# locuoco/coulomb_oscillators

Hardware: AMD Instinct MI355X
Metric: particle-steps/sec (+ Gpair-interactions/sec), N=1048576 FMM-3D kd-tree p=6, 1 GPU(s) (higher is better)
Workload: dtype f32; 1 GPU; FMM-3D kd-tree p=6, N=1048576 per GPU (one system of 1048576), leapfrog, Gaussian ball, tree rebuilt every 1 step(s); n_per_gpu=1048576, order=6, parallelism=single GPU, L=15, p2p_pairs=3193446, m2l_pairs=800719, build_mode=0, warm_builds=283, warm_misses=12, near_field=one-directional

## Files before the change

### coulomb_oscillators_amd/csrc/k_fmm_kd.hip

```cpp
#include "nbco_internal.hpp"
#include "k_p2p.hpp"
#include "kd_common.hpp"
#include <rocprim/rocprim.hpp>
#include <chrono>
#include <functional>
#include <cmath>
#include <algorithm>
#include <vector>

namespace {

using kdc::wave_scan_add;
using kdc::wave_min_u32;

constexpr int sym_off(int n) { return n * (n + 1) * (n + 2) / 6; }
constexpr int tl_off(int n) { return n * n; }

struct TreeView
{
	float *center, *lbound, *rbound;
	float4 *csz;
	float *mpole, *local;
	int *mult, *index, *splitdim;
	int L, ntot;
// ... 137 lines not shown
		hipLaunchKernelGGL(list_segsort_kernel<false>, dim3((ntargets + kBlock / 64 - 1) / (kBlock / 64)), dim3(kBlock), 0, st, (const int *)start,
		                   ntargets, keys_tmp, keys_out, shift, (const int *)nullptr, (const int *)nullptr, (int2 *)nullptr, MutualLists{}, 0);
	NBCO_HIP(hipGetLastError());
	return NBCO_OK;
}

static int kd_carve(nbco_ctx *c, DevBuf &buf, KdTreeDev &k, int ntot, int offM, int offL)
{
	const size_t rb = c->o.far_fp64 ? 8 : 4;
	k.real_bytes = (int)rb;
	size_t bytes = (size_t)ntot * (3 * 3 * sizeof(float) + sizeof(float4) + (size_t)(offM + offL) * rb + 3 * sizeof(int)) + 256 + 64;
	NBCO_TRY(c->reserve(buf, bytes));
	char *q = (char *)buf.ptr;
	k.csz = (float4 *)q; q += sizeof(float4) * (size_t)ntot;
	k.center = (float *)q; q += 12 * (size_t)ntot;
	k.lbound = (float *)q; q += 12 * (size_t)ntot;
	k.rbound = (float *)q; q += 12 * (size_t)ntot;
	q = (char *)(((uintptr_t)q + 15) & ~(uintptr_t)15);
	k.mpole = (float *)q; q += rb * (size_t)ntot * offM;
	q = (char *)(((uintptr_t)q + 15) & ~(uintptr_t)15);
	k.local = (float *)q; q += rb * (size_t)ntot * offL;
	q = (char *)(((uintptr_t)q + 15) & ~(uintptr_t)15);
	k.mult = (int *)q; q += 4 * (size_t)ntot;
	k.index = (int *)q; q += 4 * (size_t)ntot;
	k.splitdim = (int *)q;
	return NBCO_OK;
}

static int kd_build_top(nbco_ctx *c, const TreeView &tv, float4 *&pos, float4 *&pos_alt, int *&unsort, int *&unsort_alt, long long n, int l0,
                        bool use_select, bool select_ready = false, bool warm = false)
{
	hipStream_t st = c->stream;
	if (use_select && l0 > 0 && !select_ready) NBCO_TRY(kd_select_begin(c, l0));
	for (int l = 0; l < l0; ++l)
	{
		if (use_select)
			NBCO_TRY(kd_select_level(c, l, n, pos, unsort, pos_alt, unsort_alt, tv.lbound, tv.rbound, tv.splitdim, tv.index,
			                         c->counters.as<int>() + 110, warm));
		else
		{
			if (l > 0) hipLaunchKernelGGL(kd_box_kernel, dim3(grid1d(kd_cnt(l))), dim3(kBlock), 0, st, tv, pos, n, l);
			hipLaunchKernelGGL(kd_keys_kernel, dim3(grid1d(n)), dim3(kBlock), 0, st, pos, tv.splitdim + kd_beg(l), n, l,
			                   c->keys.as<uint64_t>(), c->idx.as<uint32_t>());
			NBCO_TRY(sort_pairs_u64(c, c->keys.as<uint64_t>(), c->keys_alt.as<uint64_t>(), c->idx.as<uint32_t>(), c->idx_alt.as<uint32_t>(), n, 32 + l));
			hipLaunchKernelGGL(kd_permute_kernel, dim3(grid1d(n)), dim3(kBlock), 0, st, pos, unsort, c->idx_alt.as<uint32_t>(), pos_alt, unsort_alt, n);
		}
		std::swap(pos, pos_alt);
		std::swap(unsort, unsort_alt);
	}
	if (l0 > 0 && !use_select) hipLaunchKernelGGL(kd_box_kernel, dim3(grid1d(kd_cnt(l0))), dim3(kBlock), 0, st, tv, pos, n, l0);
	NBCO_HIP(hipGetLastError());
	return NBCO_OK;
}

static int kd_reserve_particles(nbco_ctx *c, long long n)
{
	NBCO_TRY(c->reserve(c->pos4, sizeof(float4) * (size_t)n));
	NBCO_TRY(c->reserve(c->pos4_alt, sizeof(float4) * (size_t)n));
	NBCO_TRY(c->reserve(c->unsort, sizeof(int) * (size_t)n));
	NBCO_TRY(c->reserve(c->unsort_alt, sizeof(int) * (size_t)n));
	NBCO_TRY(c->reserve(c->keys, sizeof(uint64_t) * (size_t)n));
	NBCO_TRY(c->reserve(c->keys_alt, sizeof(uint64_t) * (size_t)n));
	NBCO_TRY(c->reserve(c->idx, sizeof(uint32_t) * (size_t)n));
	NBCO_TRY(c->reserve(c->idx_alt, sizeof(uint32_t) * (size_t)n));
	NBCO_TRY(c->reserve(c->counters, sizeof(int) * 128));
	return NBCO_OK;
}

static int kd_build_upward(nbco_ctx *c, const float *p, long long n, int L, const float *root6, bool &rebuild, int stage = 0)
// ... 526 lines not shown
```

### coulomb_oscillators_amd/csrc/k_kdselect.hip

```cpp
#include "nbco_internal.hpp"
#include "kd_common.hpp"

namespace {

using namespace kdc;

constexpr int kBlockBig = 1024, kBlockSmall = 256;
constexpr int kBins = 2048;
constexpr int kTieCap = 64;
constexpr int kTieWords = 8;

struct SelNode
{
	uint32_t prefix[2], r[2];
	uint32_t done_part;
	uint32_t cntL, cntR, tiecnt;
	uint32_t minR;
	uint32_t below;
};

struct SelPivot { uint32_t prefix, r, neq, need; };

__device__ inline uint32_t ld_agent_u32(const uint32_t *p) { return __hip_atomic_load(p, __ATOMIC_RELAXED, __HIP_MEMORY_SCOPE_AGENT); }

template <int BLOCK>
__device__ inline void descend(const uint32_t *__restrict__ h, int bits, SelPivot &pv, uint32_t *sh )
{
	constexpr int R = BLOCK / 64;
	constexpr int PER = kBins / BLOCK;
	uint32_t v[PER], s = 0;
#pragma unroll
	for (int q = 0; q < PER; ++q) { v[q] = ld_agent_u32(&h[threadIdx.x * PER + q]); s += v[q]; }
	const int lane = threadIdx.x & 63, w = threadIdx.x >> 6;
	uint32_t incl = s;
	for (int o = 1; o < 64; o <<= 1) { uint32_t y = __shfl_up(incl, o); if (lane >= o) incl += y; }
	__syncthreads();
	if (lane == 63) sh[w] = incl;
	__syncthreads();
	uint32_t base = 0;
	for (int q = 0; q < w; ++q) base += sh[q];
	uint32_t cum = base + incl - s;
#pragma unroll
	for (int q = 0; q < PER; ++q)
	{
		if (pv.r >= cum && pv.r < cum + v[q]) { sh[R] = threadIdx.x * PER + q; sh[R + 1] = cum; sh[R + 2] = v[q]; }
		cum += v[q];
	}
	__syncthreads();
	pv.prefix = (pv.prefix << bits) | sh[R];
	pv.r -= sh[R + 1];
	pv.neq = sh[R + 2];
// ... 559 lines not shown
				uint32_t *rec = tielist + ((size_t)(j0 + jj) * kTieCap + t) * kTieWords;
				const int a2 = anc23[jj][0], a3 = anc23[jj][1];
				const uint32_t w[7] = {ordered_bits(axis_of(p[e], sd[jj])), a2 >= 0 ? ordered_bits(axis_of(p[e], a2)) : 0u,
				                       a3 >= 0 ? ordered_bits(axis_of(p[e], a3)) : 0u, (uint32_t)org[e],
				                       __float_as_uint(p[e].x), __float_as_uint(p[e].y), __float_as_uint(p[e].z)};
#pragma unroll
				for (int q = 0; q < 7; ++q) __hip_atomic_store(&rec[q], w[q], __ATOMIC_RELAXED, __HIP_MEMORY_SCOPE_AGENT);
			}
		}
		if (cat[e] < 0) continue;
		const int q = cat[e];
		const long long dst = (q == 0 ? first[0] : (q == 1 ? first[1] : (q == 2 ? first[2] : first[3])))
		                      + (long long)((pw[e * W + wv] >> (16 * q)) & 0xFFFF) + lp[e];
		pos_out[dst] = p[e];
		unsort_out[dst] = org[e];
	}
	__shared__ uint32_t fin[2];
	PART_MARK(6);
	asm volatile("s_waitcnt vmcnt(0)" ::: "memory");
	__syncthreads();
	PART_MARK(7);
	if (threadIdx.x < 2) fin[threadIdx.x] = (j0 + threadIdx.x <= j1) ? atomicAdd(&nodes[j0 + threadIdx.x].done_part, 1u) : 0xFFFFFFFFu;
	__syncthreads();
	PART_MARK(8);
	if (threadIdx.x < 64)
		for (int jj = 0; jj < 2; ++jj)
			if (j0 + jj <= j1 && fin[jj] == chunks_of_node<CHUNK>(n, j0 + jj, m) - 1)
				ties_and_boxes(pos_out, unsort_out, lbound, rbound, splitdim, index, nodes, tielist, flag, n, l, (int)(j0 + jj),
				               (int)threadIdx.x, pvs[jj], meta[jj]);
	PART_MARK(9);
}


}

int kd_select_begin(nbco_ctx *c, int l0, bool zero, long long *words_a, long long *words_b)
{
	const size_t nodes = ((size_t)1 << l0) - 1;
	NBCO_TRY(c->reserve(c->sel_hist, sizeof(uint32_t) * 3 * nodes * kBins));
	NBCO_TRY(c->reserve(c->sel_nodes, sizeof(SelNode) * nodes));
	NBCO_TRY(c->reserve(c->sel_ties, sizeof(uint32_t) * nodes * kTieCap * kTieWords));
	if (words_a) *words_a = (long long)(3 * nodes * kBins);
	if (words_b) *words_b = (long long)(sizeof(SelNode) / sizeof(uint32_t) * nodes);
	if (zero)
	{
		NBCO_HIP(hipMemsetAsync(c->sel_hist.ptr, 0, sizeof(uint32_t) * 3 * nodes * kBins, c->stream));
		NBCO_HIP(hipMemsetAsync(c->sel_nodes.ptr, 0, sizeof(SelNode) * nodes, c->stream));
	}
	return NBCO_OK;
}

template <int BLOCK, int NP>
static void select_level_launch(nbco_ctx *c, int l, long long n, const float4 *pos_in, const int *unsort_in, float4 *pos_out, int *unsort_out,
                                float *lbound, float *rbound, int *splitdim, int *index, int *flag, int warm_drop)
{
	const int m = 1 << l;
	SelNode *nodes = c->sel_nodes.as<SelNode>() + (m - 1);
	uint32_t *hist = c->sel_hist.as<uint32_t>() + (size_t)3 * (m - 1) * kBins;
	uint32_t *ties = c->sel_ties.as<uint32_t>() + (size_t)(m - 1) * kTieCap * kTieWords;
	const int *sd_l = splitdim + (m - 1);
	hipStream_t st = c->stream;
	constexpr int CHUNK = 8 * BLOCK;
	const int gchunks = (int)((n + CHUNK - 1) / CHUNK);
	if (NP == 2 && warm_drop > 0)
	{
		constexpr int EPT = BLOCK == kBlockBig ? 4 : 8;
		const int wchunks = (int)((n + EPT * BLOCK - 1) / (EPT * BLOCK));
		hipLaunchKernelGGL((sel_hist_warm_kernel<BLOCK, EPT>), dim3(wchunks), dim3(BLOCK), 0, st, pos_in, sd_l, hist, nodes, (const float *)lbound, (const float *)rbound,
		                   n, l, warm_drop);
		hipLaunchKernelGGL((sel_partition_kernel<BLOCK, 2, true, EPT>), dim3(wchunks), dim3(BLOCK), 0, st, pos_in, unsort_in, pos_out, unsort_out, sd_l, nodes, ties, n, l,
		                   lbound, rbound, splitdim, index, flag, (const uint32_t *)hist, warm_drop, c->top_sd, c->top_root1);
		return;
	}
	hipLaunchKernelGGL((sel_hist_kernel<0, BLOCK, NP == 2>), dim3(gchunks), dim3(BLOCK), 0, st, pos_in, sd_l, hist, nodes, (const float *)lbound, (const float *)rbound, n, l);
	hipLaunchKernelGGL((sel_hist_kernel<1, BLOCK, NP == 2>), dim3(gchunks), dim3(BLOCK), 0, st, pos_in, sd_l, hist, nodes, (const float *)lbound, (const float *)rbound, n, l);
	if (NP >= 3)
		hipLaunchKernelGGL((sel_hist_kernel<2, BLOCK, false>), dim3(gchunks), dim3(BLOCK), 0, st, pos_in, sd_l, hist, nodes, (const float *)lbound, (const float *)rbound, n, l);
	hipLaunchKernelGGL((sel_partition_kernel<BLOCK, NP>), dim3(gchunks), dim3(BLOCK), 0, st, pos_in, unsort_in, pos_out, unsort_out, sd_l, nodes, ties, n, l,
	                   lbound, rbound, splitdim, index, flag, (const uint32_t *)hist, 10, c->top_sd, c->top_root1);
}

int kd_select_level(nbco_ctx *c, int l, long long n, const float4 *pos_in, const int *unsort_in, float4 *pos_out, int *unsort_out,
                    float *lbound, float *rbound, int *splitdim, int *index, int *flag, bool warm)
{
	const long long node = n >> l;
	const int np = (c->sel_three_pass || node > (1LL << 22)) ? 3 : 2;
	const bool big = node >= 8 * kBlockBig;
	int warm_drop = 0;
	if (warm && np == 2)
	{
		int lg = 0;
		while ((1LL << lg) < node) ++lg;
		warm_drop = 32 - std::max(12, std::min(22, std::max(16, lg + 6)) - 2 * c->sel_warm_coarsen);
	}
#define NBCO_SEL_ARGS c, l, n, pos_in, unsort_in, pos_out, unsort_out, lbound, rbound, splitdim, index, flag, warm_drop
	if (big)
	{
		if (np == 2) select_level_launch<kBlockBig, 2>(NBCO_SEL_ARGS);
		else select_level_launch<kBlockBig, 3>(NBCO_SEL_ARGS);
	}
	else
	{
		if (np == 2) select_level_launch<kBlockSmall, 2>(NBCO_SEL_ARGS);
		else select_level_launch<kBlockSmall, 3>(NBCO_SEL_ARGS);
	}
#undef NBCO_SEL_ARGS
	NBCO_HIP(hipGetLastError());
	return NBCO_OK;
}
```

### coulomb_oscillators_amd/csrc/nbco_api.hip

```cpp
#include "nbco_internal.hpp"
#include <chrono>
#include <cstdio>
#include <cmath>
#include <new>
#include <random>

int nbco_ctx::reserve(DevBuf &b, size_t bytes)
{
	nbco_ctx *c = this;
	if (bytes <= b.bytes) return NBCO_OK;
	if (b.ptr)
	{
		NBCO_HIP(hipStreamSynchronize(stream));
		NBCO_HIP(hipFree(b.ptr));
		b.ptr = nullptr;
		b.bytes = 0;
	}
	size_t want = bytes + bytes / 8 + 256;
	NBCO_HIP(hipMalloc(&b.ptr, want));
	b.bytes = want;
	if (poison) NBCO_HIP(hipMemsetAsync(b.ptr, 0x7f, want, stream));
	return NBCO_OK;
}

// ... 111 lines not shown
	o->list_grow = 1;
	o->far_fp64 = 0;
	o->p2p_mutual = 0;
	o->track_order = 0;
	o->stream = nullptr;
	return NBCO_OK;
}

int nbco_create(nbco_ctx **out, const nbco_opts *o)
{
	if (!out) return NBCO_ERR_ARG;
	*out = nullptr;
	nbco_ctx *c = new (std::nothrow) nbco_ctx();
	if (!c) return NBCO_ERR_HIP;
	nbco_opts def;
	nbco_opts_default(&def);
	c->o = o ? *o : def;
	int rc = check_opts(c, &c->o);
	if (rc != NBCO_OK) { delete c; return rc; }
	int ndev = 0;
	hipError_t e = hipGetDeviceCount(&ndev);
	if (e != hipSuccess || ndev <= 0)
	{
		fprintf(stderr, "nbco_create: no usable HIP device (%s)\n", e != hipSuccess ? hipGetErrorString(e) : "device count is 0");
		delete c;
		return NBCO_ERR_HIP;
	}
	if (hipGetDevice(&c->device) != hipSuccess) { delete c; return NBCO_ERR_HIP; }
	hipDeviceProp_t prop;
	if (hipGetDeviceProperties(&prop, c->device) == hipSuccess) c->num_cu = prop.multiProcessorCount;
	c->stream = (hipStream_t)c->o.stream;
	c->poison = getenv("NBCO_POISON") && atoi(getenv("NBCO_POISON")) != 0;
	if (getenv("NBCO_SEL_WARM")) c->sel_warm_enabled = atoi(getenv("NBCO_SEL_WARM")) != 0;
	if (hipMalloc(&c->small.ptr, 4096) != hipSuccess) { delete c; return NBCO_ERR_HIP; }
	c->small.bytes = 4096;
	*out = c;
	return NBCO_OK;
}

int nbco_destroy(nbco_ctx *c)
{
	if (c && getenv("NBCO_HOST_TIMING") && c->host_calls)
		fprintf(stderr, "[nbco] nbco_integrate: %lld calls, %.1f us host time per call, of which %.1f us waiting for the traversal flags\n", c->host_calls,
		        1e6 * c->host_call_s / c->host_calls, 1e6 * c->host_wait_s / c->host_calls);
	if (!c) return NBCO_OK;
	hipStreamSynchronize(c->stream);
	DevBuf *bufs[] = {&c->pos4, &c->pos4_alt, &c->part, &c->small, &c->tmp3, &c->keys, &c->keys_alt, &c->idx, &c->idx_alt,
	                  &c->unsort, &c->unsort_alt, &c->sort_tmp, &c->treebuf, &c->frontier_a, &c->frontier_b, &c->p2p_list,
	                  &c->m2l_list, &c->counters, &c->p2p_keys, &c->p2p_keys_alt, &c->m2l_keys, &c->m2l_keys_alt,
	                  &c->p2p_start, &c->m2l_start, &c->p2p_chunk_off, &c->p2p_chunks, &c->sel_hist, &c->sel_nodes, &c->sel_ties, &c->list_cnt,
	                  &c->dist_top, &c->dist_tree, &c->oct_tree, &c->oct_groups, &c->scan_tmp_aux, &c->p2p_desc, &c->trav_ctr, &c->prep_state, &c->p2p_sec, &c->p2p_react, &c->order, &c->order_alt,
	                  &c->let_sel, &c->let_have, &c->dist_pos, &c->tmp3b, &c->dpart_buf};
	if (c->aux && !c->aux_is_main) { hipStreamSynchronize(c->aux); hipStreamDestroy(c->aux); }
	if (c->ev_fork) hipEventDestroy(c->ev_fork);
	if (c->ev_join) hipEventDestroy(c->ev_join);
	if (c->ev_flags) hipEventDestroy(c->ev_flags);
	if (c->h_flags) hipHostFree(c->h_flags);
	for (DevBuf *b : bufs)
		if (b->ptr) hipFree(b->ptr);
	for (auto &t : c->timers)
		for (auto &ev : t.pending) { hipEventDestroy(ev.first); hipEventDestroy(ev.second); }
	delete c;
	return NBCO_OK;
}

int nbco_set_opts(nbco_ctx *c, const nbco_opts *o)
// ... 659 lines not shown
```

### coulomb_oscillators_amd/csrc/nbco_internal.hpp

```cpp
#pragma once
#include <hip/hip_runtime.h>
#include <cstdint>
#include <cstdio>
#include <cstring>
#include <string>
#include <vector>
#include "../../include/nbco.h"

#define NBCO_HIP(call)                                                                           \
	do {                                                                                         \
		hipError_t e_ = (call);                                                                  \
		if (e_ != hipSuccess) return c->fail_hip(e_, #call, __FILE__, __LINE__);                 \
	} while (0)

#define NBCO_HIP_M(ctx_, call)                                                                   \
	do {                                                                                         \
		hipError_t e_ = (call);                                                                  \
		if (e_ != hipSuccess) return (ctx_)->fail_hip(e_, #call, __FILE__, __LINE__);            \
	} while (0)

#define NBCO_TRY(call)                   \
	do {                                 \
		int rc_ = (call);                \
		if (rc_ != NBCO_OK) return rc_;  \
// ... 98 lines not shown
	int flags_begin();
	const int *top_sd = nullptr;
	int top_root1 = 1;
	int flags_seq = 0;
	int wait_flags();
	DevBuf scan_tmp_aux;
	int fork_aux();
	int fork_mark();
	int fork_wait();
	int join_aux();
	std::string err;
	int device = 0;
	int num_cu = 256;

	DevBuf pos4;
	DevBuf pos4_alt;
	DevBuf part;
	DevBuf small;
	DevBuf tmp3, tmp3b;
	DevBuf keys, keys_alt, idx, idx_alt, unsort, unsort_alt, sort_tmp;
	DevBuf treebuf;
	KdTreeDev kd;
	DevBuf frontier_a, frontier_b, p2p_list, m2l_list, counters;
	DevBuf p2p_keys, p2p_keys_alt, m2l_keys, m2l_keys_alt, p2p_start, m2l_start;
	DevBuf p2p_chunk_off, p2p_chunks, p2p_desc;
	DevBuf order, order_alt;
	long long order_n = -1;
	DevBuf p2p_sec, p2p_react;
	const int *pc_mult = nullptr, *pc_total = nullptr;
	int pc_shift = 0;
	DevBuf list_cnt, trav_ctr;
	DevBuf prep_state;
	DevBuf sel_hist, sel_nodes, sel_ties;
	DevBuf dist_top, dist_tree;
	DevBuf let_sel, let_have, dist_pos;
	DevBuf oct_tree, oct_groups;
	OctTreeDev oct;
	struct DistState
	{
		int world = 0, rank = 0, d = 0, L = 0;
		long long n_global = 0, n_local = 0;
		bool partitioned = false, build_done = false, local_done = false, rebuilt = false, traversed = false, let_selected = false, let_packed = false;
		const void *pos_all = nullptr;
		bool let_capped = false, let_flagged = false;
		long long let_epoch = 0;
		bool let_ignore[2] = {false, false};
	} dist;
	bool sel_warm_enabled = true, sel_warm_used = false;
	int sel_warm_coarsen = 0, sel_warm_good = 0, sel_warm_recent = 0, sel_warm_recent_miss = 0, sel_warm_cooldown = 0, sel_warm_cool_len = 128;
	long long sel_warm_builds = 0, sel_warm_misses = 0;
	void note_warm_miss()
	{
		++sel_warm_misses;
		sel_warm_good = 0;
		if (sel_warm_coarsen < 3) ++sel_warm_coarsen;
		if (++sel_warm_recent_miss >= 2)
		{
			sel_warm_cooldown = sel_warm_cool_len;
			sel_warm_cool_len = sel_warm_cool_len < 2048 ? 2 * sel_warm_cool_len : 4096;
			sel_warm_recent = sel_warm_recent_miss = 0;
		}
	}
	void note_warm_ok()
	{
		if (++sel_warm_recent >= 32) sel_warm_recent = sel_warm_recent_miss = 0;
		if (++sel_warm_good >= 64)
		{
			if (sel_warm_coarsen > 0) --sel_warm_coarsen;
			sel_warm_cool_len = sel_warm_cool_len > 256 ? sel_warm_cool_len / 2 : 128;
			sel_warm_good = 0;
		}
	}
	bool sel_three_pass = false;
	bool force_sort_build = false;
	bool escalate_build()
	{
		if (!sel_three_pass) { sel_three_pass = true; return true; }
		if (!force_sort_build) { force_sort_build = true; return true; }
		return false;
	}
	long long list_cap = 0;
// ... 72 lines not shown
int launch_energy(nbco_ctx *c, const float *buf, long long n, const float *param, double *out3_host);
int fmm_kdtree_eval(nbco_ctx *c, float *p, float *a, long long n, const float *param);
int kd_copy_out(nbco_ctx *c, int which, void *host_dst, long long host_bytes);
int kd_count_pairs(nbco_ctx *c, long long *out);
int kd_energy_fmm(nbco_ctx *c, long long n_own, double *half_phi_sum);
int launch_energy_kin_ela(nbco_ctx *c, const float *buf, long long n, const float *param, double *out2_host);
int fmm_oct_traceless_eval(nbco_ctx *c, float *p, float *a, long long n, const float *param, bool symmetric = false, int world = 1, int rank = 0,
                           long long *pbounds_host = nullptr);
int oct_copy_out(nbco_ctx *c, int which, void *host_dst, long long host_bytes);
int kd_dist_layout(nbco_ctx *c, long long n_global, int world, int rank, nbco_dist_layout *out);
int kd_dist_partition(nbco_ctx *c, const float *state_all, long long n_global, int world, int rank, float *state_local);
int dpart_workspace(nbco_ctx *c, long long n_global, int world, long long *bytes);
int dpart_begin(nbco_ctx *c, float *state_local, long long n_global, int world, int rank, void *work, long long work_bytes, nbco_dist_step *out);
int dpart_next(nbco_ctx *c, nbco_dist_step *out);
int kd_finish_pending_order(nbco_ctx *c, float *p, long long n);
int kd_turnaround(nbco_ctx *c, float *p, const float *v_in, const float **v_now, const float *param, float ks, float ds, bool elastic, long long n,
                  const float *root6 = nullptr);
int kd_dist_turnaround(nbco_ctx *c, float *buf_local, long long n_local, const float *param, float ks, float ds, bool elastic);
int kd_dist_let_select(nbco_ctx *c, const void *csz_all, long long *counts);
int kd_dist_let_pack(nbco_ctx *c, const long long *counts_all, void *pos_send, void *mpole_send);
int kd_dist_let_finish(nbco_ctx *c, const long long *counts_all, const void *pos_recv, const void *mpole_recv, float *buf_local, float *a_local, const float *param);
int kd_dist_let_check(nbco_ctx *c);
int kd_dist_let_pack_capped(nbco_ctx *c, const long long *caps_out, void *pos_send, void *mpole_send);
int kd_dist_let_finish_capped(nbco_ctx *c, const long long *caps_in, const void *pos_recv, const void *mpole_recv, float *buf_local, float *a_local, const float *param);
int kd_dist_let_settle(nbco_ctx *c, int ok);
int kd_dist_local(nbco_ctx *c, float *buf_local, long long n_local, void *nodes_send, void *pos_send, void *csz_send = nullptr,
                  void *mpole_send = nullptr, int let_stage = 0);
int kd_dist_finish(nbco_ctx *c, const void *nodes_all, const void *pos_all, float *buf_local, float *a_local, const float *param);
int kd_dist_finish_traverse(nbco_ctx *c, const void *csz_all, const void *pos_all);
int kd_dist_finish_rest(nbco_ctx *c, const void *mpole_all, float *buf_local, float *a_local, const float *param);
int kd_select_begin(nbco_ctx *c, int l0, bool zero = true, long long *words_a = nullptr, long long *words_b = nullptr);
int kd_select_level(nbco_ctx *c, int l, long long n, const float4 *pos_in, const int *unsort_in, float4 *pos_out, int *unsort_out,
                    float *lbound, float *rbound, int *splitdim, int *index, int *flag, bool warm = false);
int launch_upward_gen(nbco_ctx *c, int P, const float4 *pos, float *center, void *mpole, int *mult, const int *index, int L, int write_geom, int f64 = 0);
int launch_kd_centres(nbco_ctx *c, float *center, int *mult, int L, const float *lbound, const float *rbound, float4 *csz);
int launch_downward_gen(nbco_ctx *c, int P, const float *center, void *local, int L, int dom_d, int dom_g, int f64 = 0);
int launch_m2m_top_gen(nbco_ctx *c, int P, float *center, void *mpole, int *mult, int ltop, int L, int write_geom, int f64 = 0);
int launch_kd_centres_top(nbco_ctx *c, float *center, int *mult, int ltop, const float *lbound, const float *rbound, float4 *csz);
int launch_l2p_gen(nbco_ctx *c, int P, const float4 *pos, const float *center, const void *local, const float4 *near, const int *chunk_off,
                   const int *index, int mlt_max, const int *unsort, int scatter, const float *param, float *a, int have_near, long long n, int L,
                   long long own0, long long own_n, const int2 *sec_range = nullptr, const float4 *react = nullptr, long long react_cap = 0,
                   int react_stride = 32, int f64 = 0);
int launch_m2l_lanes(nbco_ctx *c, int P, const float4 *csz, const float *mpole, float *local, const uint64_t *keys, const int *start,
                     int shift, int ntot, int mstride = 0);
int launch_m2l_lanes_f64(nbco_ctx *c, int P, const float4 *csz, const double *mpole, double *local, const uint64_t *keys, const int *start,
                         int shift, int ntot, int mstride = 0);
```

Baseline: 486.6 million particle-steps/s.

## Fuse two kd-tree select levels per pass in warm tree builds

Adds a paired warm-select path that splits two kd-tree levels in one histogram plus partition kernel pair. Children are histogrammed using the previous build's bounds, and grandchild pivots are resolved from tie records in a tail step. This halves the number of passes over the particle array and the kernel launches during the top-level build. In exchange the kernels are much more complex, use extra record buffers, and fall back to a miss flag when the tie capacity or the predicted split axis fails.

```diff
diff --git a/coulomb_oscillators_amd/csrc/k_fmm_kd.hip b/coulomb_oscillators_amd/csrc/k_fmm_kd.hip
--- a/coulomb_oscillators_amd/csrc/k_fmm_kd.hip
+++ b/coulomb_oscillators_amd/csrc/k_fmm_kd.hip
@@ -193,9 +193,16 @@
 {
 	hipStream_t st = c->stream;
 	if (use_select && l0 > 0 && !select_ready) NBCO_TRY(kd_select_begin(c, l0));
+	const bool pair = use_select && warm && c->sel_pair_enabled;
+	if (pair) NBCO_TRY(kd_select_pair_begin(c, n, l0));
 	for (int l = 0; l < l0; ++l)
 	{
-		if (use_select)
+		if (pair && kd_select_pair_ok(c, l, n, l0))
+		{
+			NBCO_TRY(kd_select_pair(c, l, n, pos, unsort, pos_alt, unsort_alt, tv.lbound, tv.rbound, tv.splitdim, tv.index, c->counters.as<int>() + 110));
+			++l;
+		}
+		else if (use_select)
 			NBCO_TRY(kd_select_level(c, l, n, pos, unsort, pos_alt, unsort_alt, tv.lbound, tv.rbound, tv.splitdim, tv.index,
 			                         c->counters.as<int>() + 110, warm));
 		else
diff --git a/coulomb_oscillators_amd/csrc/k_kdselect.hip b/coulomb_oscillators_amd/csrc/k_kdselect.hip
--- a/coulomb_oscillators_amd/csrc/k_kdselect.hip
+++ b/coulomb_oscillators_amd/csrc/k_kdselect.hip
@@ -17,6 +17,7 @@
 	uint32_t cntL, cntR, tiecnt;
 	uint32_t minR;
 	uint32_t below;
+	uint32_t nrec;
 };
 
 struct SelPivot { uint32_t prefix, r, neq, need; };
@@ -642,6 +643,570 @@
 }
 
 
+constexpr int kPairBlock = 1024, kPairEPT = 4, kPairChunk = kPairBlock * kPairEPT;
+constexpr int kCmWords = 12;
+
+__device__ inline void warm_frame(const uint32_t *w, int drop, int &a, float &lo, float &scale, uint32_t &w0)
+{
+	a = w[0] < 3u ? (int)w[0] : 0;
+	lo = __uint_as_float(w[1 + a]);
+	const float span = __fsub_rn(__uint_as_float(w[4 + a]), lo);
+	scale = span > 0.f ? __fdiv_rn(4294967040.f, span) : 0.f;
+	const uint32_t c = lin_key(__uint_as_float(w[7 + a]), lo, scale) >> drop;
+	w0 = c > (uint32_t)(kWarmBins / 2) ? c - (uint32_t)(kWarmBins / 2) : 0u;
+}
+
+__device__ inline uint32_t old_desc_word(const int *__restrict__ splitdim, const float *__restrict__ lbound, const float *__restrict__ rbound, int node, int t)
+{
+	const int left = 2 * node + 1;
+	if (t == 0) return (uint32_t)splitdim[node];
+	if (t < 4) return __float_as_uint(lbound[3 * node + (t - 1)]);
+	if (t < 7) return __float_as_uint(rbound[3 * node + (t - 4)]);
+	if (t < 10) return __float_as_uint(rbound[3 * left + (t - 7)]);
+	return 0u;
+}
+
+template <int BLOCK, int EPT>
+__global__ __launch_bounds__(BLOCK) void sel_hist_warm_kernel_pair(const float4 *__restrict__ pos, const int *__restrict__ splitdim,
+                                                                    uint32_t *__restrict__ hist_all, SelNode *__restrict__ nodes_all,
+                                                                    uint4 *__restrict__ recs, int rec_cap, const float *__restrict__ lbound,
+                                                                    const float *__restrict__ rbound, long long n, int l, int drop, int drop1, int cpn)
+{
+	constexpr int CHUNK = EPT * BLOCK, PER = EPT;
+	__shared__ uint32_t h[3][kWarmBins];
+	__shared__ uint32_t cnt_s[4];
+	__shared__ uint32_t desc[3][kCmWords];
+	const long long m = 1LL << l;
+	const long long j = blockIdx.x / cpn;
+	const long long i0 = range_start(n, j, m) + (long long)(blockIdx.x % cpn) * CHUNK, e1 = range_start(n, j + 1, m);
+	const long long iend = i0 + CHUNK < e1 ? i0 + CHUNK : e1;
+	float4 p[PER];
+#pragma unroll
+	for (int e = 0; e < PER; ++e)
+	{
+		const long long i = i0 + e * BLOCK + threadIdx.x;
+		if (i < iend) p[e] = pos[i];
+	}
+	for (int t = threadIdx.x; t < 3 * kWarmBins; t += BLOCK) (&h[0][0])[t] = 0;
+	if (threadIdx.x < 4) cnt_s[threadIdx.x] = 0;
+	if (threadIdx.x < 3 * kCmWords)
+	{
+		const int k = threadIdx.x / kCmWords, t = threadIdx.x % kCmWords;
+		const int node = k == 0 ? (int)(m - 1 + j) : (int)(2 * m - 1 + 2 * j + (k - 1));
+		desc[k][t] = old_desc_word(splitdim, lbound, rbound, node, t);
+	}
+	__syncthreads();
+	int a[3];
+	float lo[3], scale[3];
+	uint32_t w0[3];
+#pragma unroll
+	for (int k = 0; k < 3; ++k) warm_frame(desc[k], k == 0 ? drop : drop1, a[k], lo[k], scale[k], w0[k]);
+	uint32_t nb[3] = {0, 0, 0};
+	int rslot[PER];
+#pragma unroll
+	for (int e = 0; e < PER; ++e)
+	{
+		const long long i = i0 + e * BLOCK + threadIdx.x;
+		rslot[e] = -1;
+		if (i < iend)
+		{
+			const uint32_t bj = lin_key(axis_of(p[e], a[0]), lo[0], scale[0]) >> drop;
+			if (bj - w0[0] < (uint32_t)kWarmBins)
+			{
+				atomicAdd(&h[0][bj - w0[0]], 1u);
+				rslot[e] = (int)atomicAdd(&cnt_s[3], 1u);
+			}
+			else
+			{
+				const bool r = bj >= w0[0];
+				if (!r) nb[0] += 1;
+				const int ak = r ? a[2] : a[1];
+				const uint32_t wk = r ? w0[2] : w0[1];
+				const uint32_t bc = lin_key(axis_of(p[e], ak), r ? lo[2] : lo[1], r ? scale[2] : scale[1]) >> drop1;
+				if (bc < wk) { if (r) nb[2] += 1; else nb[1] += 1; }
+				else if (bc - wk < (uint32_t)kWarmBins) atomicAdd(&h[r ? 2 : 1][bc - wk], 1u);
+			}
+		}
+	}
+#pragma unroll
+	for (int q = 0; q < 3; ++q)
+	{
+		uint32_t v = nb[q];
+		for (int o = 32; o > 0; o >>= 1) v += __shfl_xor(v, o);
+		if ((threadIdx.x & 63) == 0 && v) atomicAdd(&cnt_s[q], v);
+	}
+	__syncthreads();
+	uint32_t *hist_l = hist_all + (size_t)3 * (m - 1) * kBins, *hist_l1 = hist_all + (size_t)3 * (2 * m - 1) * kBins;
+	for (int t = threadIdx.x; t < 3 * kWarmBins; t += BLOCK)
+	{
+		const uint32_t v = (&h[0][0])[t];
+		const int k = t / kWarmBins, bin = t % kWarmBins;
+		if (!v) continue;
+		if (k == 0) atomicAdd(&hist_l[((size_t)(bin / kBins) * m + j) * kBins + (bin % kBins)], v);
+		else atomicAdd(&hist_l1[((size_t)(bin / kBins) * 2 * m + 2 * j + (k - 1)) * kBins + (bin % kBins)], v);
+	}
+	SelNode *nodes = nodes_all + (m - 1), *nodes1 = nodes_all + (2 * m - 1);
+	__shared__ uint32_t rbase;
+	if (threadIdx.x == 0) rbase = cnt_s[3] ? atomicAdd(&nodes[j].nrec, cnt_s[3]) : 0u;
+	else if (threadIdx.x == 1 && cnt_s[0]) atomicAdd(&nodes[j].below, cnt_s[0]);
+	else if (threadIdx.x < 4 && cnt_s[threadIdx.x - 1]) atomicAdd(&nodes1[2 * j + (threadIdx.x - 2)].below, cnt_s[threadIdx.x - 1]);
+	__syncthreads();
+#pragma unroll
+	for (int e = 0; e < PER; ++e)
+	{
+		if (rslot[e] < 0) continue;
+		const uint32_t r = rbase + (uint32_t)rslot[e];
+		if (r >= (uint32_t)rec_cap) continue;
+		const uint32_t bj = lin_key(axis_of(p[e], a[0]), lo[0], scale[0]) >> drop;
+		const uint32_t b1 = lin_key(axis_of(p[e], a[1]), lo[1], scale[1]) >> drop1, b2 = lin_key(axis_of(p[e], a[2]), lo[2], scale[2]) >> drop1;
+		recs[(size_t)j * rec_cap + r] = make_uint4(bj, b1, b2, 0u);
+	}
+}
+
+template <int BLOCK>
+__device__ inline bool band_find(const uint32_t *h, uint32_t rlo, uint32_t rhi, uint32_t *sh , uint32_t &blo, uint32_t &bhi)
+{
+	constexpr int R = BLOCK / 64, PER = kWarmBins / BLOCK;
+	uint32_t v[PER], s = 0;
+#pragma unroll
+	for (int q = 0; q < PER; ++q) { v[q] = h[threadIdx.x * PER + q]; s += v[q]; }
+	const int lane = threadIdx.x & 63, w = threadIdx.x >> 6;
+	const uint32_t incl = wave_scan_add(s);
+	__syncthreads();
+	if (lane == 63) sh[w] = incl;
+	if (threadIdx.x == 0) { sh[R] = 0xFFFFFFFFu; sh[R + 1] = 0xFFFFFFFFu; }
+	__syncthreads();
+	const uint32_t wt = lane < R ? sh[lane] : 0u;
+	uint32_t cum = __shfl(wave_scan_add(wt) - wt, w) + incl - s;
+#pragma unroll
+	for (int q = 0; q < PER; ++q)
+	{
+		if (rlo >= cum && rlo < cum + v[q]) sh[R] = threadIdx.x * PER + q;
+		if (rhi >= cum && rhi < cum + v[q]) sh[R + 1] = threadIdx.x * PER + q;
+		cum += v[q];
+	}
+	__syncthreads();
+	blo = sh[R]; bhi = sh[R + 1];
+	__syncthreads();
+	return blo != 0xFFFFFFFFu && bhi != 0xFFFFFFFFu;
+}
+
+__device__ inline void next_axes(const uint32_t *chain, int len, int a1, int &a2, int &a3)
+{
+	a2 = -1; a3 = -1;
+	for (int t = 0; t < len; ++t)
+	{
+		const int a = (int)chain[t];
+		if (a > 2) break;
+		if (a == a1 || a == a2) continue;
+		if (a2 < 0) a2 = a;
+		else { a3 = a; break; }
+	}
+}
+
+#pragma clang fp contract(off)
+__device__ inline uint32_t cand_rank(uint32_t nt, uint32_t k1, uint32_t k2, uint32_t k3, uint32_t org)
+{
+	uint32_t rank = 0;
+	for (uint32_t q = 0; q < nt; ++q)
+	{
+		const uint32_t q1 = __shfl(k1, q), q2 = __shfl(k2, q), q3 = __shfl(k3, q), qo = __shfl(org, q);
+		const bool before = q1 < k1 || (q1 == k1 && (q2 < k2 || (q2 == k2 && (q3 < k3 || (q3 == k3 && qo < org)))));
+		rank += before ? 1u : 0u;
+	}
+	return rank;
+}
+__device__ inline void set_axis(float (&v)[3], int a, float x)
+{
+	if (a == 0) v[0] = x; else if (a == 1) v[1] = x; else v[2] = x;
+}
+__device__ inline void write_node(float *__restrict__ lbound, float *__restrict__ rbound, int *__restrict__ splitdim, int *__restrict__ index,
+                                  int node, const float *lb, const float *rb, long long first)
+{
+	lbound[3 * node] = lb[0]; lbound[3 * node + 1] = lb[1]; lbound[3 * node + 2] = lb[2];
+	rbound[3 * node] = rb[0]; rbound[3 * node + 1] = rb[1]; rbound[3 * node + 2] = rb[2];
+	splitdim[node] = longest_axis(rb[0] - lb[0], rb[1] - lb[1], rb[2] - lb[2]);
+	index[node] = (int)first;
+}
+
+struct PairHead
+{
+	SelPivot pv;
+	bool missj, missc[2];
+	int a, ac[2];
+	float loc[2], scc[2];
+	uint32_t blo[2], bhi[2];
+	int a23[2], c23[2][2];
+};
+
+__device__ inline void pair_tail(float4 *__restrict__ pos_out, int *__restrict__ unsort_out, float *__restrict__ lbound, float *__restrict__ rbound,
+                                 int *__restrict__ splitdim, int *__restrict__ index, SelNode *__restrict__ nodes, SelNode *__restrict__ nodes1,
+                                 const uint32_t *__restrict__ ties, const uint32_t *__restrict__ ties1, int *__restrict__ flag, long long n, int l,
+                                 int j, int lane, const PairHead &hd, const uint32_t *meta, int drop1)
+{
+	const long long m = 1LL << l;
+	const int a = hd.a;
+	const uint64_t lower = (1ull << lane) - 1ull;
+	float cl0[3], cr0[3], cl1[3], cr1[3];
+#pragma unroll
+	for (int q = 0; q < 3; ++q) { cl0[q] = cl1[q] = __uint_as_float(meta[kMetaLb + q]); cr0[q] = cr1[q] = __uint_as_float(meta[kMetaRb + q]); }
+	bool missj = hd.missj, mc[2] = {hd.missc[0], hd.missc[1]};
+	bool mine = false, left = false;
+	float4 pp = make_float4(0.f, 0.f, 0.f, 0.f);
+	uint32_t porg = 0;
+	if (!missj)
+	{
+		const uint32_t *rec = ties + ((size_t)j * kTieCap + lane) * kTieWords;
+		const uint32_t nt = ld_agent_u32(&nodes[j].tiecnt), inv = ld_agent_u32(&nodes[j].minR);
+		const uint32_t k1 = ld_agent_u32(rec), k2 = ld_agent_u32(rec + 1), k3 = ld_agent_u32(rec + 2), org = ld_agent_u32(rec + 3);
+		const uint32_t bx = ld_agent_u32(rec + 4), by = ld_agent_u32(rec + 5), bz = ld_agent_u32(rec + 6);
+		if (nt > kTieCap || nt < hd.pv.need) missj = true;
+		else
+		{
+			mine = (uint32_t)lane < nt;
+			const uint32_t rank = cand_rank(nt, k1, k2, k3, org);
+			left = rank < hd.pv.need;
+			pp = make_float4(__uint_as_float(bx), __uint_as_float(by), __uint_as_float(bz), 0.f);
+			porg = org;
+			const unsigned long long at_pivot = __ballot(mine && rank + 1 == hd.pv.need), after = __ballot(mine && rank == hd.pv.need);
+			const uint32_t pivot = __shfl(k1, __ffsll((long long)at_pivot) - 1);
+			const uint32_t cand_right = after ? __shfl(k1, __ffsll((long long)after) - 1) : 0xFFFFFFFFu;
+			const uint32_t above = inv ? ~inv : 0xFFFFFFFFu;
+			set_axis(cr0, a, unordered_bits(pivot));
+			set_axis(cl1, a, unordered_bits(cand_right < above ? cand_right : above));
+		}
+	}
+	if (missj) { mc[0] = mc[1] = true; }
+	if (longest_axis(cr0[0] - cl0[0], cr0[1] - cl0[1], cr0[2] - cl0[2]) != hd.ac[0]) mc[0] = true;
+	if (longest_axis(cr1[0] - cl1[0], cr1[1] - cl1[1], cr1[2] - cl1[2]) != hd.ac[1]) mc[1] = true;
+	if (lane == 0) write_node(lbound, rbound, splitdim, index, (int)(2 * m - 1 + 2 * j), cl0, cr0, range_start(n, 2 * j, 2 * m));
+	if (lane == 1) write_node(lbound, rbound, splitdim, index, (int)(2 * m - 1 + 2 * j + 1), cl1, cr1, range_start(n, 2 * j + 1, 2 * m));
+#pragma unroll
+	for (int k = 0; k < 2; ++k)
+	{
+		const long long c = 2 * j + k;
+		float gl0[3], gr0[3], gl1[3], gr1[3];
+#pragma unroll
+		for (int q = 0; q < 3; ++q) { gl0[q] = gl1[q] = k ? cl1[q] : cl0[q]; gr0[q] = gr1[q] = k ? cr1[q] : cr0[q]; }
+		if (!mc[k])
+		{
+			const int ac = hd.ac[k];
+			const long long gL = range_start(n, 2 * c, 4 * m), gR = range_start(n, 2 * c + 1, 4 * m);
+			const uint32_t ntc = ld_agent_u32(&nodes1[c].tiecnt), cL = ld_agent_u32(&nodes1[c].cntL), cR = ld_agent_u32(&nodes1[c].cntR);
+			const uint32_t invc = ld_agent_u32(&nodes1[c].minR);
+			const uint32_t *rec = ties1 + ((size_t)c * kTieCap + lane) * kTieWords;
+			uint32_t k1 = ld_agent_u32(rec), k2 = ld_agent_u32(rec + 1), k3 = ld_agent_u32(rec + 2), org = ld_agent_u32(rec + 3);
+			uint32_t bx = ld_agent_u32(rec + 4), by = ld_agent_u32(rec + 5), bz = ld_agent_u32(rec + 6);
+			const bool pk = mine && (left == (k == 0));
+			const float xk = axis_of(pp, ac);
+			const uint32_t bc = lin_key(xk, hd.loc[k], hd.scc[k]) >> drop1;
+			const unsigned long long bpb = __ballot(pk && bc < hd.blo[k]), bpa = __ballot(pk && bc > hd.bhi[k]);
+			const unsigned long long bpi = __ballot(pk && bc >= hd.blo[k] && bc <= hd.bhi[k]);
+			const uint32_t PB = (uint32_t)__popcll(bpb), PA = (uint32_t)__popcll(bpa), PI = (uint32_t)__popcll(bpi);
+			const uint32_t kx = ordered_bits(xk);
+			if ((bpb >> lane) & 1ull) { const long long d = gL + cL + __popcll(bpb & lower); pos_out[d] = pp; unsort_out[d] = (int)porg; }
+			if ((bpa >> lane) & 1ull) { const long long d = gR + cR + __popcll(bpa & lower); pos_out[d] = pp; unsort_out[d] = (int)porg; }
+			const uint32_t minA = wave_min_u32(((bpa >> lane) & 1ull) ? kx : 0xFFFFFFFFu);
+			const uint32_t nt = ntc + PI;
+			if (ntc > kTieCap || nt > kTieCap) mc[k] = true;
+			else
+			{
+				int src = lane;
+				unsigned long long bits = bpi;
+				for (uint32_t t = 0; t < PI; ++t)
+				{
+					const int b = __ffsll((long long)bits) - 1;
+					if ((uint32_t)lane == ntc + t) src = b;
+					bits &= bits - 1ull;
+				}
+				const int c2 = hd.c23[k][0], c3 = hd.c23[k][1];
+				const uint32_t pk1 = kx, pk2 = c2 >= 0 ? ordered_bits(axis_of(pp, c2)) : 0u, pk3 = c3 >= 0 ? ordered_bits(axis_of(pp, c3)) : 0u;
+				const uint32_t s1 = __shfl(pk1, src), s2 = __shfl(pk2, src), s3 = __shfl(pk3, src), so = __shfl(porg, src);
+				const uint32_t sx = __shfl(__float_as_uint(pp.x), src), sy = __shfl(__float_as_uint(pp.y), src), sz = __shfl(__float_as_uint(pp.z), src);
+				if ((uint32_t)lane >= ntc) { k1 = s1; k2 = s2; k3 = s3; org = so; bx = sx; by = sy; bz = sz; }
+				const bool cm = (uint32_t)lane < nt;
+				const uint32_t rank = cand_rank(nt, k1, k2, k3, org);
+				const long long below = (long long)cL + PB, rc = gR - range_start(n, c, 2 * m) - 1;
+				const long long need = rc + 1 - below;
+				if (need < 1 || need > (long long)nt) mc[k] = true;
+				else
+				{
+					if (cm)
+					{
+						const long long d = (long long)rank < need ? gL + below + rank : gR + cR + PA + (rank - need);
+						pos_out[d] = make_float4(__uint_as_float(bx), __uint_as_float(by), __uint_as_float(bz), 0.f);
+						unsort_out[d] = (int)org;
+					}
+					const unsigned long long at_pivot = __ballot(cm && rank + 1 == need), after = __ballot(cm && rank == need);
+					const uint32_t pivot = __shfl(k1, __ffsll((long long)at_pivot) - 1);
+					const uint32_t cand_right = after ? __shfl(k1, __ffsll((long long)after) - 1) : 0xFFFFFFFFu;
+					uint32_t rmin = invc ? ~invc : 0xFFFFFFFFu;
+					rmin = minA < rmin ? minA : rmin;
+					rmin = cand_right < rmin ? cand_right : rmin;
+					set_axis(gr0, ac, unordered_bits(pivot));
+					set_axis(gl1, ac, unordered_bits(rmin));
+				}
+			}
+		}
+		if (lane == 0) write_node(lbound, rbound, splitdim, index, (int)(4 * m - 1 + 2 * c), gl0, gr0, range_start(n, 2 * c, 4 * m));
+		if (lane == 1) write_node(lbound, rbound, splitdim, index, (int)(4 * m - 1 + 2 * c + 1), gl1, gr1, range_start(n, 2 * c + 1, 4 * m));
+	}
+	if (lane == 0 && (missj || mc[0] || mc[1])) *flag = 2;
+}
+#pragma clang fp contract(on)
+
+template <int BLOCK, int EPT>
+__global__ __launch_bounds__(BLOCK) void sel_partition_kernel_pair(const float4 *__restrict__ pos_in, const int *__restrict__ unsort_in,
+                                                                    float4 *__restrict__ pos_out, int *__restrict__ unsort_out,
+                                                                    SelNode *__restrict__ nodes_all, uint32_t *__restrict__ ties_all,
+                                                                    const uint4 *__restrict__ recs, int rec_cap, long long n, int l,
+                                                                    float *__restrict__ lbound, float *__restrict__ rbound, int *__restrict__ splitdim,
+                                                                    int *__restrict__ index, int *__restrict__ flag, const uint32_t *__restrict__ hist_all,
+                                                                    int drop, int drop1, int cpn, const int *__restrict__ top_sd, int top_root1)
+{
+	constexpr int CHUNK = EPT * BLOCK, PER = EPT, W = BLOCK / 64;
+	static_assert(CHUNK < 65536, "packed 16-bit block counters");
+	const long long m = 1LL << l;
+	const long long j = blockIdx.x / cpn;
+	const long long i0 = range_start(n, j, m) + (long long)(blockIdx.x % cpn) * CHUNK, e1 = range_start(n, j + 1, m);
+	const long long iend = i0 + CHUNK < e1 ? i0 + CHUNK : e1;
+	SelNode *nodes = nodes_all + (m - 1), *nodes1 = nodes_all + (2 * m - 1);
+	uint32_t *ties = ties_all + (size_t)(m - 1) * kTieCap * kTieWords;
+	uint32_t *ties1 = ties_all + (size_t)(2 * m - 1) * kTieCap * kTieWords;
+	const uint32_t *hist_l = hist_all + (size_t)3 * (m - 1) * kBins, *hist_l1 = hist_all + (size_t)3 * (2 * m - 1) * kBins;
+	const uint4 *rj = recs + (size_t)j * rec_cap;
+	float4 p[PER];
+	int org[PER];
+#pragma unroll
+	for (int e = 0; e < PER; ++e)
+	{
+		const long long i = i0 + e * BLOCK + threadIdx.x;
+		if (i < iend) { p[e] = pos_in[i]; org[e] = unsort_in[i]; }
+	}
+	__shared__ uint32_t meta[kMetaWords];
+	__shared__ uint32_t cm[2][kCmWords];
+	__shared__ uint32_t hc[2][kWarmBins];
+	__shared__ uint32_t ntie_s[3], mR[3], xb_s[2], base_s[7];
+	constexpr int kMetaRec = kMetaBelow + 1;
+	if (threadIdx.x < 64)
+	{
+		const int t = threadIdx.x, node = (int)(m - 1 + j), left = 2 * node + 1;
+		uint32_t v = 0;
+		if (t < 32)
+		{
+			v = 3u;
+			if (t < l) v = (uint32_t)splitdim[(((int)(m + j)) >> (t + 1)) - 1];
+			else if (top_sd) { const int up = top_root1 >> (t - l + 1); if (up > 0) v = (uint32_t)top_sd[up - 1]; }
+		}
+		else if (t == kMetaSd) v = (uint32_t)splitdim[node];
+		else if (t < kMetaRb) v = __float_as_uint(lbound[3 * node + (t - kMetaLb)]);
+		else if (t < kMetaOld) v = __float_as_uint(rbound[3 * node + (t - kMetaRb)]);
+		else if (t < kMetaBelow) v = __float_as_uint(rbound[3 * left + (t - kMetaOld)]);
+		else if (t == kMetaBelow) v = ld_agent_u32(&nodes[j].below);
+		else if (t == kMetaRec) v = ld_agent_u32(&nodes[j].nrec);
+		meta[t] = v;
+	}
+	else if (threadIdx.x < 64 + 2 * kCmWords)
+	{
+		const int k = (threadIdx.x - 64) / kCmWords, t = (threadIdx.x - 64) % kCmWords;
+		const int c = (int)(2 * j + k);
+		cm[k][t] = t < 10 ? old_desc_word(splitdim, lbound, rbound, (int)(2 * m - 1) + c, t) : (t == 10 ? ld_agent_u32(&nodes1[c].below) : 0u);
+	}
+	for (int t = threadIdx.x; t < 2 * kWarmBins; t += BLOCK)
+	{
+		const int k = t / kWarmBins, bin = t % kWarmBins;
+		(&hc[0][0])[t] = ld_agent_u32(&hist_l1[((size_t)(bin / kBins) * 2 * m + 2 * j + k) * kBins + (bin % kBins)]);
+	}
+	uint32_t wbins[kWarmBins / BLOCK];
+	warm_bins<BLOCK>(hist_l, m, j, wbins);
+	uint4 rv[2];
+#pragma unroll
+	for (int q = 0; q < 2; ++q)
+	{
+		const int r = threadIdx.x + q * BLOCK;
+		rv[q] = r < rec_cap ? rj[r] : make_uint4(0, 0, 0, 0);
+	}
+	if (threadIdx.x < 3) { ntie_s[threadIdx.x] = 0; mR[threadIdx.x] = 0xFFFFFFFFu; }
+	if (threadIdx.x < 2) xb_s[threadIdx.x] = 0;
+	__syncthreads();
+	__shared__ uint32_t sh[BLOCK / 64 + 4];
+	PairHead hd;
+	float loj, scj;
+	uint32_t w0j, w0c[2];
+	warm_frame(&meta[kMetaSd], drop, hd.a, loj, scj, w0j);
+#pragma unroll
+	for (int k = 0; k < 2; ++k) warm_frame(cm[k], drop1, hd.ac[k], hd.loc[k], hd.scc[k], w0c[k]);
+	next_axes(meta, 32, hd.a, hd.a23[0], hd.a23[1]);
+#pragma unroll
+	for (int k = 0; k < 2; ++k)
+	{
+		int a2 = -1, a3 = -1;
+		const int ac = hd.ac[k];
+		if (hd.a != ac) a2 = hd.a;
+		for (int t = 0; t < 32 && a3 < 0; ++t)
+		{
+			const int x = (int)meta[t];
+			if (x > 2) break;
+			if (x == ac || x == a2) continue;
+			if (a2 < 0) a2 = x; else a3 = x;
+		}
+		hd.c23[k][0] = a2; hd.c23[k][1] = a3;
+	}
+	hd.pv = resolve_warm<BLOCK>(wbins, meta[kMetaBelow], n, l, j, w0j, sh);
+	const uint32_t nrec = meta[kMetaRec];
+	hd.missj = hd.pv.need == 0 || nrec > (uint32_t)rec_cap;
+	const uint32_t B = hd.pv.prefix;
+	if (!hd.missj)
+	{
+		for (uint32_t r = threadIdx.x; r < nrec; r += BLOCK)
+		{
+			const uint4 v = r < (uint32_t)BLOCK ? rv[0] : (r < 2u * BLOCK ? rv[1] : rj[r]);
+			if (v.x == B) continue;
+			const int k = v.x < B ? 0 : 1;
+			const uint32_t b = k ? v.z : v.y, wk = k ? w0c[1] : w0c[0];
+			if (b < wk) atomicAdd(&xb_s[k], 1u);
+			else if (b - wk < (uint32_t)kWarmBins) atomicAdd(&hc[k][b - wk], 1u);
+		}
+	}
+	__syncthreads();
+#pragma unroll
+	for (int k = 0; k < 2; ++k)
+	{
+		hd.missc[k] = hd.missj;
+		hd.blo[k] = hd.bhi[k] = 0;
+		const long long c = 2 * j + k;
+		const long long rc = range_start(n, 2 * c + 1, 4 * m) - range_start(n, c, 2 * m) - 1;
+		const long long q = k == 0 ? (long long)hd.pv.need : (long long)hd.pv.neq - (long long)hd.pv.need;
+		const long long bel = (long long)cm[k][10] + xb_s[k];
+		const bool ok = !hd.missj && rc >= q + bel;
+		uint32_t blo = 0, bhi = 0;
+		const bool found = band_find<BLOCK>(hc[k], ok ? (uint32_t)(rc - q - bel) : 0u, ok ? (uint32_t)(rc - bel) : 0u, sh, blo, bhi);
+		hd.missc[k] = !ok || !found;
+		hd.blo[k] = w0c[k] + blo; hd.bhi[k] = w0c[k] + bhi;
+	}
+	__shared__ uint64_t pw[PER * W + 1];
+	const int wv = threadIdx.x >> 6, lane = threadIdx.x & 63;
+	const uint64_t lower = (1ull << lane) - 1ull;
+	int cat[PER], tlist[PER], tslot[PER];
+	uint32_t lp[PER];
+	uint32_t tmin[3] = {0xFFFFFFFFu, 0xFFFFFFFFu, 0xFFFFFFFFu};
+#pragma unroll
+	for (int e = 0; e < PER; ++e)
+	{
+		const long long i = i0 + e * BLOCK + threadIdx.x;
+		cat[e] = -1; tlist[e] = -1; tslot[e] = -1;
+		if (i < iend && !hd.missj)
+		{
+			const float xa = axis_of(p[e], hd.a);
+			const uint32_t bj = lin_key(xa, loj, scj) >> drop;
+			if (bj == B) tlist[e] = 0;
+			else
+			{
+				const bool r = bj > B;
+				if (r) { const uint32_t key = ordered_bits(xa); tmin[0] = key < tmin[0] ? key : tmin[0]; }
+				if (!(r ? hd.missc[1] : hd.missc[0]))
+				{
+					const float xc = axis_of(p[e], r ? hd.ac[1] : hd.ac[0]);
+					const uint32_t bc = lin_key(xc, r ? hd.loc[1] : hd.loc[0], r ? hd.scc[1] : hd.scc[0]) >> drop1;
+					if (bc < (r ? hd.blo[1] : hd.blo[0])) cat[e] = r ? 2 : 0;
+					else if (bc > (r ? hd.bhi[1] : hd.bhi[0]))
+					{
+						cat[e] = r ? 3 : 1;
+						const uint32_t key = ordered_bits(xc);
+						if (r) tmin[2] = key < tmin[2] ? key : tmin[2];
+						else tmin[1] = key < tmin[1] ? key : tmin[1];
+					}
+					else tlist[e] = r ? 2 : 1;
+				}
+			}
+			if (tlist[e] >= 0) tslot[e] = (int)atomicAdd(&ntie_s[tlist[e]], 1u);
+		}
+		uint64_t packed = 0;
+		lp[e] = 0;
+#pragma unroll
+		for (int q = 0; q < 4; ++q)
+		{
+			const uint64_t bq = __ballot(cat[e] == q);
+			packed |= (uint64_t)__popcll(bq) << (16 * q);
+			if (cat[e] == q) lp[e] = (uint32_t)__popcll(bq & lower);
+		}
+		if (lane == 0) pw[e * W + wv] = packed;
+	}
+#pragma unroll
+	for (int q = 0; q < 3; ++q)
+	{
+		const uint32_t v = wave_min_u32(tmin[q]);
+		if (lane == 0 && v != 0xFFFFFFFFu) atomicMin(&mR[q], v);
+	}
+	__syncthreads();
+	if (threadIdx.x < 64)
+	{
+		constexpr int NE = PER * W;
+		const int k0 = 2 * lane, k1 = 2 * lane + 1;
+		const uint64_t v0 = k0 < NE ? pw[k0] : 0, v1 = k1 < NE ? pw[k1] : 0;
+		const uint64_t both = v0 + v1;
+		const uint64_t incl = (uint64_t)wave_scan_add((uint32_t)both) | ((uint64_t)wave_scan_add((uint32_t)(both >> 32)) << 32);
+		const uint64_t excl = incl - both;
+		if (k0 < NE) pw[k0] = excl;
+		if (k1 < NE) pw[k1] = excl + v0;
+		const uint64_t tot = __shfl(incl, 63);
+		if (lane < 4)
+		{
+			const uint32_t c = (uint32_t)((tot >> (16 * lane)) & 0xFFFF);
+			SelNode &cn = nodes1[2 * j + (lane >> 1)];
+			base_s[lane] = c ? atomicAdd((lane & 1) ? &cn.cntR : &cn.cntL, c) : 0;
+		}
+		else if (lane < 7)
+		{
+			const uint32_t c = ntie_s[lane - 4];
+			base_s[lane] = c ? atomicAdd(lane == 4 ? &nodes[j].tiecnt : &nodes1[2 * j + (lane - 5)].tiecnt, c) : 0;
+		}
+		else if (lane < 10)
+		{
+			const uint32_t v = mR[lane - 7];
+			if (v != 0xFFFFFFFFu) atomicMax(lane == 7 ? &nodes[j].minR : &nodes1[2 * j + (lane - 8)].minR, ~v);
+		}
+	}
+	__syncthreads();
+	long long first[4];
+#pragma unroll
+	for (int q = 0; q < 4; ++q) first[q] = range_start(n, 4 * j + q, 4 * m) + base_s[q];
+#pragma unroll
+	for (int e = 0; e < PER; ++e)
+	{
+		if (tslot[e] >= 0)
+		{
+			const int tl = tlist[e];
+			const uint32_t t = base_s[4 + tl] + (uint32_t)tslot[e];
+			if (t < kTieCap)
+			{
+				uint32_t *rec = tl == 0 ? ties + ((size_t)j * kTieCap + t) * kTieWords : ties1 + ((size_t)(2 * j + tl - 1) * kTieCap + t) * kTieWords;
+				const int a1 = tl == 0 ? hd.a : (tl == 1 ? hd.ac[0] : hd.ac[1]);
+				const int a2 = tl == 0 ? hd.a23[0] : (tl == 1 ? hd.c23[0][0] : hd.c23[1][0]);
+				const int a3 = tl == 0 ? hd.a23[1] : (tl == 1 ? hd.c23[0][1] : hd.c23[1][1]);
+				const uint32_t w[7] = {ordered_bits(axis_of(p[e], a1)), a2 >= 0 ? ordered_bits(axis_of(p[e], a2)) : 0u,
+				                       a3 >= 0 ? ordered_bits(axis_of(p[e], a3)) : 0u, (uint32_t)org[e],
+				                       __float_as_uint(p[e].x), __float_as_uint(p[e].y), __float_as_uint(p[e].z)};
+#pragma unroll
+				for (int q = 0; q < 7; ++q) __hip_atomic_store(&rec[q], w[q], __ATOMIC_RELAXED, __HIP_MEMORY_SCOPE_AGENT);
+			}
+		}
+		if (cat[e] < 0) continue;
+		const int q = cat[e];
+		const long long dst = (q == 0 ? first[0] : (q == 1 ? first[1] : (q == 2 ? first[2] : first[3])))
+		                      + (long long)((pw[e * W + wv] >> (16 * q)) & 0xFFFF) + lp[e];
+		pos_out[dst] = p[e];
+		unsort_out[dst] = org[e];
+	}
+	__shared__ uint32_t fin;
+	asm volatile("s_waitcnt vmcnt(0)" ::: "memory");
+	__syncthreads();
+	if (threadIdx.x == 0) fin = atomicAdd(&nodes[j].done_part, 1u);
+	__syncthreads();
+	if (threadIdx.x < 64 && fin == (uint32_t)cpn - 1)
+		pair_tail(pos_out, unsort_out, lbound, rbound, splitdim, index, nodes, nodes1, ties, ties1, flag, n, l, (int)j, (int)threadIdx.x, hd, meta, drop1);
+}
+
 }
 
 int kd_select_begin(nbco_ctx *c, int l0, bool zero, long long *words_a, long long *words_b)
@@ -690,19 +1255,20 @@
 	                   lbound, rbound, splitdim, index, flag, (const uint32_t *)hist, 10, c->top_sd, c->top_root1);
 }
 
+static int warm_drop_of(const nbco_ctx *c, long long node)
+{
+	int lg = 0;
+	while ((1LL << lg) < node) ++lg;
+	return 32 - std::max(12, std::min(22, std::max(16, lg + 6)) - 2 * c->sel_warm_coarsen);
+}
+
 int kd_select_level(nbco_ctx *c, int l, long long n, const float4 *pos_in, const int *unsort_in, float4 *pos_out, int *unsort_out,
                     float *lbound, float *rbound, int *splitdim, int *index, int *flag, bool warm)
 {
 	const long long node = n >> l;
 	const int np = (c->sel_three_pass || node > (1LL << 22)) ? 3 : 2;
 	const bool big = node >= 8 * kBlockBig;
-	int warm_drop = 0;
-	if (warm && np == 2)
-	{
-		int lg = 0;
-		while ((1LL << lg) < node) ++lg;
-		warm_drop = 32 - std::max(12, std::min(22, std::max(16, lg + 6)) - 2 * c->sel_warm_coarsen);
-	}
+	const int warm_drop = warm && np == 2 ? warm_drop_of(c, node) : 0;
 #define NBCO_SEL_ARGS c, l, n, pos_in, unsort_in, pos_out, unsort_out, lbound, rbound, splitdim, index, flag, warm_drop
 	if (big)
 	{
@@ -718,3 +1284,44 @@
 	NBCO_HIP(hipGetLastError());
 	return NBCO_OK;
 }
+
+bool kd_select_pair_ok(const nbco_ctx *c, int l, long long n, int l0)
+{
+	return l + 1 < l0 && !c->sel_three_pass && (n >> l) <= (1LL << 22);
+}
+
+int kd_select_pair_begin(nbco_ctx *c, long long n, int l0)
+{
+	long long off = 0;
+	for (int l = 0; l < l0 && l < 32; ++l)
+	{
+		const long long node = n >> l;
+		const int drop = warm_drop_of(c, node);
+		const long long expect = ((long long)kWarmBins * (node + 1)) >> (32 - drop);
+		long long cap = 1024;
+		while (cap < 8 * expect || (cap < 4096 && cap < node / 4)) cap <<= 1;
+		c->sel_rec_off[l] = off;
+		c->sel_rec_cap[l] = (int)cap;
+		off += cap << l;
+	}
+	return c->reserve(c->sel_recs, sizeof(uint4) * (size_t)off);
+}
+
+int kd_select_pair(nbco_ctx *c, int l, long long n, const float4 *pos_in, const int *unsort_in, float4 *pos_out, int *unsort_out,
+                   float *lbound, float *rbound, int *splitdim, int *index, int *flag)
+{
+	const long long m = 1LL << l;
+	const int drop = warm_drop_of(c, n >> l), drop1 = warm_drop_of(c, n >> (l + 1));
+	const int cpn = (int)(((n + m - 1) / m + kPairChunk - 1) / kPairChunk);
+	const int grid = (int)(m * cpn);
+	uint4 *recs = c->sel_recs.as<uint4>() + c->sel_rec_off[l];
+	const int cap = c->sel_rec_cap[l];
+	hipStream_t st = c->stream;
+	hipLaunchKernelGGL((sel_hist_warm_kernel_pair<kPairBlock, kPairEPT>), dim3(grid), dim3(kPairBlock), 0, st, pos_in, (const int *)splitdim,
+	                   c->sel_hist.as<uint32_t>(), c->sel_nodes.as<SelNode>(), recs, cap, (const float *)lbound, (const float *)rbound, n, l, drop, drop1, cpn);
+	hipLaunchKernelGGL((sel_partition_kernel_pair<kPairBlock, kPairEPT>), dim3(grid), dim3(kPairBlock), 0, st, pos_in, unsort_in, pos_out, unsort_out,
+	                   c->sel_nodes.as<SelNode>(), c->sel_ties.as<uint32_t>(), (const uint4 *)recs, cap, n, l, lbound, rbound, splitdim, index, flag,
+	                   (const uint32_t *)c->sel_hist.as<uint32_t>(), drop, drop1, cpn, c->top_sd, c->top_root1);
+	NBCO_HIP(hipGetLastError());
+	return NBCO_OK;
+}
diff --git a/coulomb_oscillators_amd/csrc/nbco_api.hip b/coulomb_oscillators_amd/csrc/nbco_api.hip
--- a/coulomb_oscillators_amd/csrc/nbco_api.hip
+++ b/coulomb_oscillators_amd/csrc/nbco_api.hip
@@ -167,6 +167,7 @@
 	c->stream = (hipStream_t)c->o.stream;
 	c->poison = getenv("NBCO_POISON") && atoi(getenv("NBCO_POISON")) != 0;
 	if (getenv("NBCO_SEL_WARM")) c->sel_warm_enabled = atoi(getenv("NBCO_SEL_WARM")) != 0;
+	if (getenv("NBCO_SEL_PAIR")) c->sel_pair_enabled = atoi(getenv("NBCO_SEL_PAIR")) != 0;
 	if (hipMalloc(&c->small.ptr, 4096) != hipSuccess) { delete c; return NBCO_ERR_HIP; }
 	c->small.bytes = 4096;
 	*out = c;
diff --git a/coulomb_oscillators_amd/csrc/nbco_internal.hpp b/coulomb_oscillators_amd/csrc/nbco_internal.hpp
--- a/coulomb_oscillators_amd/csrc/nbco_internal.hpp
+++ b/coulomb_oscillators_amd/csrc/nbco_internal.hpp
@@ -154,6 +154,9 @@
 	DevBuf list_cnt, trav_ctr;
 	DevBuf prep_state;
 	DevBuf sel_hist, sel_nodes, sel_ties;
+	DevBuf sel_recs;
+	long long sel_rec_off[32] = {};
+	int sel_rec_cap[32] = {};
 	DevBuf dist_top, dist_tree;
 	DevBuf let_sel, let_have, dist_pos;
 	DevBuf oct_tree, oct_groups;
@@ -169,6 +172,7 @@
 		bool let_ignore[2] = {false, false};
 	} dist;
 	bool sel_warm_enabled = true, sel_warm_used = false;
+	bool sel_pair_enabled = true;
 	int sel_warm_coarsen = 0, sel_warm_good = 0, sel_warm_recent = 0, sel_warm_recent_miss = 0, sel_warm_cooldown = 0, sel_warm_cool_len = 128;
 	long long sel_warm_builds = 0, sel_warm_misses = 0;
 	void note_warm_miss()
@@ -307,6 +311,10 @@
 int kd_select_begin(nbco_ctx *c, int l0, bool zero = true, long long *words_a = nullptr, long long *words_b = nullptr);
 int kd_select_level(nbco_ctx *c, int l, long long n, const float4 *pos_in, const int *unsort_in, float4 *pos_out, int *unsort_out,
                     float *lbound, float *rbound, int *splitdim, int *index, int *flag, bool warm = false);
+int kd_select_pair_begin(nbco_ctx *c, long long n, int l0);
+bool kd_select_pair_ok(const nbco_ctx *c, int l, long long n, int l0);
+int kd_select_pair(nbco_ctx *c, int l, long long n, const float4 *pos_in, const int *unsort_in, float4 *pos_out, int *unsort_out,
+                   float *lbound, float *rbound, int *splitdim, int *index, int *flag);
 int launch_upward_gen(nbco_ctx *c, int P, const float4 *pos, float *center, void *mpole, int *mult, const int *index, int L, int write_geom, int f64 = 0);
 int launch_kd_centres(nbco_ctx *c, float *center, int *mult, int L, const float *lbound, const float *rbound, float4 *csz);
 int launch_downward_gen(nbco_ctx *c, int P, const float *center, void *local, int L, int dom_d, int dom_g, int f64 = 0);
```

Measured after the change: 488.1 million particle-steps/s (median of 6 runs). About the same (+0.3%).
